# Dylan-H-Wang/skin-sm3

Measured on AMD Instinct MI355X. Metric: SM3 pretrain images/sec (paired 224x224), higher is better.
Workload: dtype bf16

## Files before the change

include/sm3_hip.h:

```cpp
#ifndef SM3_HIP_H
#define SM3_HIP_H

#include <stdint.h>

#ifdef __cplusplus
extern "C" {
#endif

#define SM3_F32 0
#define SM3_BF16 1
#define SM3_F16 2

#define SM3_EINVAL (-1)
#define SM3_EALIGN (-2)
#define SM3_EDTYPE (-3)

#define SM3_MAX_TAPS 9

int sm3_abi_version(void);

typedef struct sm3_conv_desc {
    int32_t dtype;
    int32_t N, Hi, Wi, Ci;
    int32_t Ho, Wo, Co;
// ... 68 lines not shown
                    float* save_invstd , void* stream);
int sm3_bn_eval_scale_shift(const float* gamma, const float* beta, const float* running_mean,
                            const float* running_var, float eps, int C, float* scale, float* shift,
                            void* stream);
int sm3_bn_act(int dtype, const void* x, const float* scale, const float* shift, const void* residual,
               int relu, int out_f32, void* y, uint8_t* relu_mask, int64_t rows, int C, int views, void* stream);
int sm3_bn_act_colsum_rows(int64_t rows, int C, int dtype);
int sm3_bn_act_colsum(int dtype, const void* x, const float* scale, const float* shift, const void* residual, int relu,
                      void* y, uint8_t* relu_mask, float* colsum_partials, int64_t rows, int C, int views, void* stream);
int sm3_subsample_colsum_rows(int64_t rows, int C, int dtype);
int sm3_subsample_colsum(int dtype, const void* x, void* y, float* colsum_partials, int N, int H, int W, int C, int stride,
                         int views, void* stream);
int sm3_bn_add_bn_act(int dtype, const void* x, const float* scale, const float* shift, const void* x2,
                      const float* scale2, const float* shift2, int relu, void* y, uint8_t* relu_mask,
                      int64_t rows, int C, int views, void* stream);
int sm3_bn_bwd_partial_rows(int64_t rows, int C);
int sm3_bn_bwd_reduce(int dtype, const void* dy, const void* y, const uint8_t* relu_mask, const void* x,
                      const float* mean, const float* invstd, void* dz, int64_t rows, int C,
                      float* partials , int views, void* stream);
int sm3_bn_bwd_apply(int dtype, const void* dz, const void* x, const float* mean, const float* invstd,
                     const float* gamma, const double* global_sums, double count,
                     const double* local_sums, float* dgamma, float* dbeta, void* dx, int64_t rows,
                     int C, int views, void* stream);

typedef struct sm3_bn_apply_side {
    const void* x;
    const float* mean;
    const float* invstd;
    const float* gamma;
    const double* global_sums;
    const double* local_sums;
    float* dgamma;
    float* dbeta;
    void* dx;
} sm3_bn_apply_side;
int sm3_bn_bwd_apply2(int dtype, const void* dz, double count, const sm3_bn_apply_side* a,
                      const sm3_bn_apply_side* b, int64_t rows, int C, int views, void* stream);

int sm3_linbn_moments(const float* slabs, int nslabs, int64_t n, float* out, const float* colsum_partials, int colsum_rows,
                      double* s_out, int p, int views, void* stream);
int sm3_linbn_fwd_stats(int dtype, const float* G, const void* w_dgrad, const void* w_fwd, const double* s, float* Tm,
                        double* sums_ws, int C, int p, int views, void* stream);
int sm3_linbn_stats(int dtype, const float* P, const void* w_fwd, const float* mean, const float* invstd, const float* gamma,
                    const double* reduce_ws, int groups, double* lsums, float* dgamma, float* dbeta, double count,
                    float* coef, int C, int p, int views, void* stream);
int sm3_linbn_coef(const double* global_sums, double count, const float* gamma, const float* mean, const float* invstd,
// ... 232 lines not shown
```

skin-sm3_amd/csrc/bn.hip:

```cpp
#include "common.h"
#include <cstdlib>

namespace {

struct RowWalk {
    int tbx, tby;
    int gx, gy;
};
static RowWalk make_walk(int64_t rows, int cvecs, int max_gy, int views = 1) {
    RowWalk w;
    if (cvecs >= 256) {
        w.tbx = 256;
    } else {
        w.tbx = cvecs;
    }
    w.tby = 256 / w.tbx;
    if (w.tby < 1) w.tby = 1;
    w.gx = (cvecs + w.tbx - 1) / w.tbx;
    int64_t gy = (rows + (int64_t)w.tby * 8 - 1) / ((int64_t)w.tby * 8);
    static const int grid_cap = getenv("SM3_BN_GRID_CAP") ? atoi(getenv("SM3_BN_GRID_CAP")) : 768;
    const int64_t cap = grid_cap / (w.gx * views) > 0 ? grid_cap / (w.gx * views) : 1;
    if (gy > cap) gy = cap;
    if (gy > max_gy) gy = max_gy;
    if (gy < 1) gy = 1;
// ... 40 lines not shown
    double a = (a0 + a1) + (a2 + a3);
    a += __shfl_xor(a, 1, 64);
    a += __shfl_xor(a, 2, 64);
    return a;
}

__global__ void bn_stats_reduce_b(const double* __restrict__ ws, int G, int C, double* __restrict__ sums) {
    ws += (long)blockIdx.z * G * 2 * C;
    sums += (long)blockIdx.z * 2 * C;
    const int t = blockIdx.x * blockDim.x + threadIdx.x, q = t & 3;
    const int col = t >> 2;
    const double a = quad_sum_groups(ws, 2L * C, col < 2 * C ? col : 0, G, q);
    if (col < 2 * C && q == 0) sums[col] = a;
}

struct BnFinalizeArgs {
    double count;
    int C;
    const float *gamma, *beta;
    float eps, momentum;
    float *running_mean, *running_var;
    float *scale, *shift, *save_mean, *save_invstd;
};
__device__ __forceinline__ void bn_finalize_channel(const double* __restrict__ sums, int groups, int views, int c, int lane16,
                                                    const BnFinalizeArgs& a) {
    const int C = a.C;
    const int q = lane16 & 3, stat = (lane16 >> 2) & 1, vl = (lane16 >> 3) & 1;
    const int cc = c < C ? c : 0;
    float rm = 0.f, rv = 0.f;
    const bool owner = (c < C) && (lane16 == 0);
    if (owner) {
        rm = a.running_mean ? a.running_mean[c] : 0.f;
        rv = a.running_var ? a.running_var[c] : 0.f;
    }
    for (int v0 = 0; v0 < views; v0 += 2) {
        const int v = v0 + vl;
        const bool vok = v < views;
        const double* sv = sums + (long)(vok ? v : v0) * groups * 2 * C;
        const double mine = quad_sum_groups(sv, 2L * C, (long)stat * C + cc, groups, q);
        const double s2_same_view = __shfl_down(mine, 4, 64);
        const double s1_v1 = __shfl_down(mine, 8, 64);
        const double s2_v1 = __shfl_down(mine, 12, 64);
        if (!owner) continue;
        for (int k = 0; k < 2 && v0 + k < views; ++k) {
            const double s1 = k ? s1_v1 : mine, s2 = k ? s2_v1 : s2_same_view;
            const int vv = v0 + k;
            const double mean = s1 / a.count;
            double var = s2 / a.count - mean * mean;
            if (var < 0) var = 0;
            const double invstd = 1.0 / sqrt(var + (double)a.eps);
            const float g = a.gamma ? a.gamma[c] : 1.f, b = a.beta ? a.beta[c] : 0.f;
            a.scale[(long)vv * C + c] = (float)(g * invstd);
            a.shift[(long)vv * C + c] = (float)((double)b - mean * (double)g * invstd);
            if (a.save_mean) a.save_mean[(long)vv * C + c] = (float)mean;
            if (a.save_invstd) a.save_invstd[(long)vv * C + c] = (float)invstd;
            rm = (1.f - a.momentum) * rm + a.momentum * (float)mean;
            const double unbiased = var * (a.count / fmax(a.count - 1.0, 1.0));
            rv = (1.f - a.momentum) * rv + a.momentum * (float)unbiased;
        }
    }
    if (owner) {
        if (a.running_mean) a.running_mean[c] = rm;
        if (a.running_var) a.running_var[c] = rv;
    }
}

__global__ void bn_finalize_kernel(const double* __restrict__ sums, int groups, int views, int64_t* nbt, BnFinalizeArgs a) {
    const int t = blockIdx.x * blockDim.x + threadIdx.x;
    if (t == 0 && nbt) nbt[0] += views;
    bn_finalize_channel(sums, groups, views, t >> 4, t & 15, a);
}

__global__ void bn_eval_kernel(const float* gamma, const float* beta, const float* rm, const float* rv, float eps,
                               int C, float* scale, float* shift) {
    const int c = blockIdx.x * blockDim.x + threadIdx.x;
    if (c >= C) return;
    const float invstd = 1.f / sqrtf(rv[c] + eps);
    const float g = gamma ? gamma[c] : 1.f, b = beta ? beta[c] : 0.f;
    scale[c] = g * invstd;
    shift[c] = b - rm[c] * g * invstd;
}
// ... 427 lines not shown
        for (int e = 0; e < E; ++e) o[e] = k0a[e] * (g[e] - k1a[e]) - (xv[e] - mua[e]) * qa[e];
        stg16<NT>(dxa + r * C + (int64_t)cv * E, pack16<T>(o));
        unpack16<T>(xbu, xv);
#pragma unroll
        for (int e = 0; e < E; ++e) o[e] = k0b[e] * (g[e] - k1b[e]) - (xv[e] - mub[e]) * qb[e];
        stg16<NT>(dxb + r * C + (int64_t)cv * E, pack16<T>(o));
    };
    int64_t r = (int64_t)blockIdx.y * tby + ty;
    for (; r + (U - 1) * rstep < rows; r += U * rstep) {
        uint4 gu[U], xau[U], xbu[U];
#pragma unroll
        for (int u = 0; u < U; ++u) {
            const int64_t off = (r + u * rstep) * C + (int64_t)cv * E;
            gu[u] = ldg16<NT>(dz + off);
            xau[u] = ldg16<NT>(xa + off);
            xbu[u] = ldg16<NT>(xb + off);
        }
#pragma unroll
        for (int u = 0; u < U; ++u) finish(r + u * rstep, gu[u], xau[u], xbu[u]);
    }
    for (; r < rows; r += rstep) {
        const int64_t off = r * C + (int64_t)cv * E;
        finish(r, ldg16<false>(dz + off), ldg16<false>(xa + off), ldg16<false>(xb + off));
    }
}

static int env_int(const char* name, int dflt) {
    const char* v = getenv(name);
    return v && *v ? atoi(v) : dflt;
}
static int bn_unroll(int kind) {
    static const int u[3] = {env_int("SM3_BN_UNROLL_ACT", env_int("SM3_BN_UNROLL", 4)),
                             env_int("SM3_BN_UNROLL_RED", env_int("SM3_BN_UNROLL", 4)),
                             env_int("SM3_BN_UNROLL_APP", env_int("SM3_BN_UNROLL", 8))};
    return u[kind];
}
static bool bn_nt() {
    static const bool nt = env_int("SM3_BN_NT", 1) != 0;
    return nt;
}
#define SM3_BN_DISPATCH(KIND, CALL)                 \
    do {                                            \
        const int u_ = bn_unroll(KIND);             \
        if (bn_nt()) {                              \
            if (u_ >= 8) { CALL(8, true); }         \
            else if (u_ >= 4) { CALL(4, true); }    \
// ... 209 lines not shown
    for (const sm3_bn_apply_side* s : {a, b})
        if (!s->x || !s->mean || !s->invstd || !s->global_sums || !s->dx) return SM3_EINVAL;
    if (!SM3_DTYPE_OK(dtype)) return SM3_EDTYPE;
    const int E = dtype == SM3_F32 ? 4 : 8;
    if (C % E) return SM3_EALIGN;
    const RowWalk w = make_walk(rows, C / E, 8192, views);
    dim3 grid(w.gx, w.gy, views), block(256);
    hipStream_t st = (hipStream_t)stream;
    const BnApplySide sa = {a->x, a->mean, a->invstd, a->gamma, a->global_sums, a->local_sums, a->dgamma, a->dbeta, a->dx};
    const BnApplySide sb = {b->x, b->mean, b->invstd, b->gamma, b->global_sums, b->local_sums, b->dgamma, b->dbeta, b->dx};
#define SM3_APP2_T(T, U, NT)                                                                                   \
    hipLaunchKernelGGL((bn_bwd_apply2_kernel<T, (U > 4 ? 4 : U), NT>), grid, block, 0, st, (const T*)dz, sa, sb,  \
                       1.0 / count, rows, C, w.tbx, w.tby)
#define SM3_APP2(U, NT)                                        \
    if (dtype == SM3_F32) { SM3_APP2_T(float, U, NT); }        \
    else if (dtype == SM3_BF16) { SM3_APP2_T(bf16_t, U, NT); } \
    else { SM3_APP2_T(f16_t, U, NT); }
    SM3_BN_DISPATCH(2, SM3_APP2);
#undef SM3_APP2
#undef SM3_APP2_T
    SM3_CHECK_LAUNCH();
    return 0;
}
```

skin-sm3_amd/sm3hip/_lib.py:

```python
import ctypes as C
import os

_HERE = os.path.dirname(os.path.abspath(__file__))
LIB_PATH = os.environ.get("SM3_LIBRARY") or os.path.join(_HERE, "libsm3hip.so")

SM3_F32, SM3_BF16, SM3_F16 = 0, 1, 2
MAX_TAPS = 9


class ConvDesc(C.Structure):
    _fields_ = [
        ("dtype", C.c_int32),
        ("N", C.c_int32), ("Hi", C.c_int32), ("Wi", C.c_int32), ("Ci", C.c_int32),
        ("Ho", C.c_int32), ("Wo", C.c_int32), ("Co", C.c_int32),
        ("sy", C.c_int32), ("sx", C.c_int32),
        ("ntaps", C.c_int32),
        ("dy", C.c_int32 * MAX_TAPS), ("dx", C.c_int32 * MAX_TAPS), ("wtap", C.c_int32 * MAX_TAPS),
        ("w_row_stride", C.c_int32),
        ("Hout", C.c_int32), ("Wout", C.c_int32),
        ("osy", C.c_int32), ("osx", C.c_int32), ("ooy", C.c_int32), ("oox", C.c_int32),
    ]


class BnBwdFuse(C.Structure):
# ... 52 lines not shown
    "sm3_linbn_stats": [_I, _P, _P, _P, _P, _P, _P, _I, _P, _P, _P, _D, _P, _I, _I, _I, _P],
    "sm3_linbn_coef": [_P, _D, _P, _P, _P, _P, _I, _I, _P],
    "sm3_linbn_banks": [_I, _P, _P, _P, _P, _P, _I, _I, _I, _P],
    "sm3_linbn_post": [_I, _P, _P, _P, _P, _P, _P, _P, _P, _P, _I, _I, _I, _P],
    "sm3_linbn_banks_post": [_I, _P, _P, _P, _P, _P, _P, _P, _P, _P, _P, _I, _I, _I, _P],
    "sm3_conv_bn_act_eval": [_DESC, _P, _P, _P, _P, _P, _I, _P, _P],
    "sm3_conv_bn_eval": [_DESC, _P, _P, _P, _P, _P, _P, _F, _P, _I, _P, _P],
    "sm3_conv_wgrad": [_DESC, _P, _P, _P, _P],
    "sm3_conv_wgrad_det": [_DESC, _P, _P, _P, _P, _I, _P],
    "sm3_slab_reduce": [_P, _I, _L, _P, _I, _P],
    "sm3_bn_stats_reduce": [_P, _I, _I, _P, _P, _I, _P],
    "sm3_bn_reduce_groups": [_I],
    "sm3_bn_finalize": [_P, _I, _I, _D, _I, _P, _P, _F, _F, _P, _P, _P, _P, _P, _P, _P, _P],
    "sm3_bn_eval_scale_shift": [_P, _P, _P, _P, _F, _I, _P, _P, _P],
    "sm3_bn_act": [_I, _P, _P, _P, _P, _I, _I, _P, _P, _L, _I, _I, _P],
    "sm3_bn_add_bn_act": [_I, _P, _P, _P, _P, _P, _P, _I, _P, _P, _L, _I, _I, _P],
    "sm3_bn_bwd_apply2": [_I, _P, _D, _P, _P, _L, _I, _I, _P],
    "sm3_bn_relu_maxpool_fwd": [_I, _P, _P, _P, _P, _P, _I, _I, _I, _I, _I, _P],
    "sm3_maxpool_bn_bwd_partial_rows": [_I, _I, _I, _I],
    "sm3_maxpool_bn_bwd": [_I, _P, _P, _P, _P, _P, _P, _P, _P, _P, _I, _I, _I, _I, _I, _P],
    "sm3_bn_bwd_partial_rows": [_L, _I],
    "sm3_bn_bwd_reduce": [_I, _P, _P, _P, _P, _P, _P, _P, _L, _I, _P, _I, _P],
    "sm3_bn_bwd_apply": [_I, _P, _P, _P, _P, _P, _P, _D, _P, _P, _P, _P, _L, _I, _I, _P],
    "sm3_stem_partial_rows": [_I, _I, _I],
    "sm3_stem_weight_prep": [_I, _P, _P, _P],
    "sm3_stem_weight_prep_if": [_I, _P, _P, _P, _P],
    "sm3_stem_conv_fwd": [_I, _P, _P, _P, _P, _I, _I, _I, _P],
    "sm3_stem_wgrad_bn": [_I, _P, _P, _P, _P, _P, _P, _P, _D, _P, _P, _P, _P, _P, _I, _I, _I, _I, _P],
    "sm3_stem_image_cols": [_I],
    "sm3_stem_image_prep": [_I, _P, _P, _P, _I, _I, _I, _I, _P],
    "sm3_stem_conv_fwd16": [_I, _P, _P, _P, _P, _I, _I, _I, _P],
    "sm3_stem_wgrad_bn16": [_I, _P, _P, _P, _P, _P, _P, _P, _D, _P, _P, _P, _P, _P, _I, _I, _I, _I, _P],
    "sm3_stem_dgrad_bn": [_I, _P, _P, _P, _P, _P, _P, _D, _P, _P, _I, _I, _I, _I, _P],
    "sm3_maxpool3x3s2_fwd": [_I, _P, _P, _P, _I, _I, _I, _I, _P],
    "sm3_maxpool3x3s2_bwd": [_I, _P, _P, _P, _I, _I, _I, _I, _P],
    "sm3_weight_prep_batch": [_I, _P, _I, _P],
    "sm3_weight_prep_batch_if": [_I, _P, _I, _P, _P],
    "sm3_weights_changed": [_P, _L, _P, _P, _P],
    "sm3_avgpool_fwd": [_I, _P, _P, _P, _I, _I, _I, _P],
    "sm3_avgpool_bwd": [_I, _P, _P, _I, _I, _I, _P],
    "sm3_weight_prep": [_I, _P, _I, _I, _I, _P, _I, _P, _P],
    "sm3_cast_from_f32": [_I, _P, _P, _L, _P],
    "sm3_cast_to_f32": [_I, _P, _P, _L, _P],
    "sm3_ntxent_logits": [_P, _I, _I, _F, _P, _P, _P, _P],
    "sm3_ntxent_logits_bwd": [_I, _P, _P, _P, _I, _I, _F, _P, _P],
    "sm3_ce_label0": [_P, _I, _I, _F, _P, _P, _P, _P],
# ... 106 lines not shown
```

skin-sm3_amd/sm3hip/engine.py:

```python
import os
from collections import OrderedDict
from contextlib import contextmanager

import torch

from . import ops
from ._lib import SM3_BF16, SM3_F16
from .plan import (TWO_PASS, BlockRec, EncoderCtx, ParamStore, ProjectorPlan, Rec, block_form, enc_mod_out_dim, enc_plan,
                   stage_of)
from .plan import EncoderPlan

BN_EPS = 1e-5
BN_MOMENTUM = 0.1


_LANE_POOL = {}


def lane_stream_pool(device, n):
    idx = device.index if device.index is not None else torch.cuda.current_device()
    pool = _LANE_POOL.setdefault(idx, [])
    if len(pool) >= n:
        return pool[:n]
    if os.environ.get("SM3_STREAM_CALIBRATE", "1") == "0" or not hasattr(torch.cuda, "_sleep"):
# ... 74 lines not shown
        self._lane = "main"
        self._V = 1
        self._data_only = False
        self._no_stat_update = False
        self.weights_dirty = True
        self._wprep_cache, self._wprep_key, self._hash_tracks_banks = {}, None, False
        self._lane_prep = {}
        self._lin_descs = {}
        self.last_feats = None
        self._faith_saved_bytes = {}
        self.pair_views = os.environ.get("SM3_PAIR_VIEWS", "1") != "0"
        self.two_streams = True
        self._streams, self._streams_dev = None, None
        self.linbn = self.dtype in (SM3_BF16, SM3_F16) and os.environ.get("SM3_LINBN", "1") != "0"
        self.linbn_fwd = os.environ.get("SM3_LINBN_FWD", "1") != "0"
        self.linbn_ds = os.environ.get("SM3_LINBN_DS", "1") != "0"
        self.linbn_join = os.environ.get("SM3_LINBN_JOIN", "1") != "0"
        self.linbn_merge = os.environ.get("SM3_LINBN_MERGE", "1") != "0"
        self.lane_cross = os.environ.get("SM3_LANE_CROSS", "1") != "0"
        if self.cross is not None and self.cross[0] is self.cross[1]:
            self.lane_cross = False
        self.det_wgrad = os.environ.get("SM3_WGRAD_DET", "1") != "0"
        self.stem16 = self.dtype in (SM3_BF16, SM3_F16) and os.environ.get("SM3_STEM16", "1") != "0"

    def _all_conv_units(self):
        seen = set()
        plans = [p for pair in self.branches.values() for p in pair if p is not None]
        plans += list(self.cross or ())
        if self.meta is not None:
            plans.append(self.meta)
        for plan in plans:
            for cu in plan.conv_units():
                if id(cu) not in seen:
                    seen.add(id(cu))
                    yield cu

    def prepare(self, device):
        if self.store is None or self.store.flat_p.device != device:
            self.store = ParamStore(self.module, device)
            self._allocated = False
        else:
            self.store.rebind_if_needed()
        if not self._allocated:
            for cu in self._all_conv_units():
                cu.alloc(self.dtype, device)
            self._allocated = True
# ... 130 lines not shown
            rm, rv = self.buffers[bu.name + ".running_mean"], self.buffers[bu.name + ".running_var"]
            nbt = self.buffers[bu.name + ".num_batches_tracked"]
        ops.bn_finalize(sums, count, bu.C, gamma, beta, BN_EPS, BN_MOMENTUM, rm, rv, nbt, scale, shift, mean, invstd,
                        groups=groups, views=V)

    @contextmanager
    def _views(self, V):
        self._V = V
        try:
            yield
        finally:
            self._V = 1

    @contextmanager
    def _params_backward(self, params):
        prev = self._data_only
        self._data_only = prev or not params
        try:
            yield
        finally:
            self._data_only = prev

    def conv_bn(self, cu, bu, x, N, H, W, relu, residual=None, train=True, save=False, out_f32=False, y_out=None,
                apply=True, scale_shift=None, res_affine=None, pending=None, colsum=None):
        dev = x.t.device if isinstance(x, ops.StemImage) else x.device
        direct = cu.stem
        if direct:
            d = None
            Ho, Wo = (H - 1) // 2 + 1, (W - 1) // 2 + 1
        else:
            d = cu.fwd_desc(self.dtype, N, H, W)
            Ho, Wo = d.Ho, d.Wo
        rows = N * Ho * Wo
        C = cu.Co
        V = self._V if train else 1
        rows_v = rows // V
        xo = torch.empty(rows, C, dtype=self.tdt, device=dev)
        scale, shift = scale_shift if scale_shift is not None else (self._work("scale", 2 * 2048),
                                                                    self._work("shift", 2 * 2048))
        mean = invstd = None

        def convolve(partials):
            if direct:
                (ops.stem_conv_fwd16 if isinstance(x, ops.StemImage) else ops.stem_conv_fwd)(self.dtype, x, cu.w_fwd, xo, partials)
            elif cu.groups > 1:
                ops.gconv_fwd(self.dtype, x, cu.w_fwd, xo, partials, N, H, W, C, cu.groups, cu.stride)
            else:
                ops.conv_gemm(d, x, cu.w_fwd, xo, None, partials)
        if train:
            prow = ops.stem_partial_rows(N, H, W) if direct else ops.conv_partial_rows(d)
            if V > 1 and ((rows_v % 128 and not direct) or prow % V):
                raise ValueError("two views in one batch need a multiple of 128 rows per view")
            partials = self._work("partials", prow * 2 * C)
            convolve(partials)
            count, groups = rows_v, 1
            mean = torch.empty(V * C, dtype=torch.float32, device=dev)
            invstd = torch.empty(V * C, dtype=torch.float32, device=dev)
            deferred = False
            if self.stat_sync is not None:
                count = rows_v * self.world_size
                n = V * 2 * C
                if pending is not None and not apply:
                    pair = self._work("sums_pair", 2 * 2 * 2 * 2048, torch.float64)
                    sums = pair[:n]
                    ops.bn_stats_reduce(partials, prow // V, C, sums, views=V)
                    deferred = True
                elif pending:
                    pair = self._work("sums_pair", 2 * 2 * 2 * 2048, torch.float64)
                    n0 = pending[0][0]
                    sums = pair[n0:n0 + n]
                    ops.bn_stats_reduce(partials, prow // V, C, sums, views=V)
                    self.stat_sync(pair[: n0 + n])
                    for _, fin in pending:
                        fin()
                    del pending[:]
                else:
                    sums = self._work("sums", 2 * 2 * 2048, torch.float64)
# ... 23 lines not shown
        mask = None
        if not apply:
            y_out = None
        else:
            if y_out is None:
                y_out = torch.empty(rows, C, dtype=torch.float32 if out_f32 else self.tdt, device=dev)
            if save and relu:
                mask = torch.empty(rows * C // (16 // ops._sz(self.dtype)), dtype=torch.uint8, device=dev)
            cs = None
            if res_affine is not None:
                ops.bn_add_bn_act(self.dtype, xo, scale, shift, residual, res_affine[0], res_affine[1], relu, y_out,
                                  rows_v, C, mask=mask, views=V)
            else:
                if colsum is not None and save and train and not out_f32:
                    cs = colsum
                ops.bn_act(self.dtype, xo, scale, shift, residual, relu, y_out, rows_v, C, out_f32=out_f32, mask=mask,
                           views=V, colsum=cs)
        r = None
        if save:
            r = Rec(cu, bu, N, H, W, Ho, Wo, x_in=x, xo=xo, mean=mean, invstd=invstd, y=y_out, relu=relu, mask=mask, V=V,
                    frozen_stats=not train, colsum=cs if apply else None)
        return (y_out if apply else xo), Ho, Wo, r

    def _phase1(self, r, dy, fused_rows):
        if fused_rows is not None:
            return fused_rows, self._ws[(self._lane, "fz_partials")]
        C, V = r.cu.Co, r.V
        rows = r.N * r.Ho * r.Wo // V
        prow = ops.bn_bwd_partial_rows(rows, C)
        bpart = self._work("partials", V * prow * 2 * C)
        ops.bn_bwd_reduce(self.dtype, dy, None, r.xo, r.mean, r.invstd, dy if r.relu else None, rows, C, bpart,
                          mask=r.mask if r.relu else None, views=V)
        return prow, bpart

    def bn_backward(self, r, dy, keep_dz, fused_rows=None):
        C = r.cu.Co
        V = r.V
        rows = r.xo.shape[0] // V
        prow, bpart = self._phase1(r, dy, fused_rows)
        lsums, gsums, count = self._bn_backward_sums(r, bpart, prow)
        dxo = torch.empty_like(r.xo) if keep_dz else dy
        dgamma, dbeta = self._bn_affine(r.bu, grad=True)
        ops.bn_bwd_apply(self.dtype, dy, r.xo, r.mean, r.invstd, self._bn_affine(r.bu)[0], gsums, count, lsums, dgamma, dbeta,
                         dxo, rows, C, views=V)
        return dxo, dy

    def _bn_backward_sums(self, r, bpart, prow):
        C, V = r.cu.Co, r.V
        rows = r.xo.shape[0] // V
        lsums = self._work("lsums", 2 * 2 * 2048, torch.float64)
        ops.bn_stats_reduce(bpart, prow, C, lsums, views=V)
        gsums, count = lsums, rows
        if r.frozen_stats:
            gsums = self._work("zsums", 2 * 2 * 2048, torch.float64)
            gsums.zero_()
        elif self.stat_sync is not None:
            gsums = self._work("gsums", 2 * 2 * 2048, torch.float64)
            gsums[: V * 2 * C].copy_(lsums[: V * 2 * C])
            self.stat_sync(gsums[: V * 2 * C])
            count = rows * self.world_size
        return lsums, gsums, count
# ... 500 lines not shown
            dd = cd.compact_dgrad_desc(self.dtype, rd.N, rd.Ho, rd.Wo)
            if cd.stride == 2:
                dsp = torch.empty(rd.N * rd.Ho * rd.Wo, Cin, dtype=self.tdt, device=dcur.device)
                ops.conv_gemm_seg(dd, dcur, dxd["wa"], dxd["x1"], dxd["hn"], dxd["const"], dsp, None, views=rd.V,
                                  w_view_stride=Cin * Cd, w1_view_stride=Cin * Cin)
                return self.conv_backward(r1, dx1, addend=dsp, fuse=prev, addend_sparse=(rd.Ho, rd.Wo))
            din, _ = self.conv_backward(r1, dx1)
            ops.conv_gemm_seg(dd, dcur, dxd["wa"], dxd["x1"], dxd["hn"], dxd["const"], din, din, views=rd.V,
                              w_view_stride=Cin * Cd, w1_view_stride=Cin * Cin)
            return din, None
        if br.form.sparse_join and prev is not None:
            self._wgrad(cd, rd, dxd)
            hs, ws = rd.Ho, rd.Wo
            dd = cd.compact_dgrad_desc(self.dtype, rd.N, hs, ws)
            dsp = torch.empty(rd.N * hs * ws, cd.Ci, dtype=self.tdt, device=dxd.device)
            ops.conv_gemm(dd, dxd, cd.w_dgrad, dsp, None, None)
            return self.conv_backward(r1, dx1, addend=dsp, fuse=prev, addend_sparse=(hs, ws))
        din, _ = self.conv_backward(r1, dx1)
        self.conv_backward(rd, dxd, into=din)
        return din, None

    def projector_forward(self, plan, x_t, M, train, z_out, save=None):
        saving = save is not None
        h, _, _, r0 = self.conv_bn(plan.l0, plan.b1, x_t, M, 1, 1, True, None, train, saving)
        h, _, _, r3 = self.conv_bn(plan.l3, plan.b4, h, M, 1, 1, True, None, train, saving)
        r6 = self.conv_bn(plan.l6, plan.b7, h, M, 1, 1, False, None, train, saving, out_f32=True, y_out=z_out)[3]
        if saving:
            save.append((r0, r3, r6))

    def projector_backward(self, recs, dz, addend=None, into=None):
        r0, r3, r6 = recs
        dx, _ = self.bn_backward(r6, dz, keep_dz=False)
        d, fr = self.conv_backward(r6, dx, fuse=r3)
        dx, _ = self.bn_backward(r3, d, keep_dz=False, fused_rows=fr)
        d, fr = self.conv_backward(r3, dx, fuse=r0)
        dx, _ = self.bn_backward(r0, d, keep_dz=False, fused_rows=fr)
        if into is not None:
            return self.conv_backward(r0, dx, into=into)[0]
        return self.conv_backward(r0, dx, addend=addend)[0]

    @staticmethod
    def cross_pairs(style):
        return {0: [(0, 0), (1, 1)], 1: [(0, 1), (1, 0)], 2: [(0, 0), (0, 1), (1, 0), (1, 1)]}[style]

    def forward(self, views, style=0, train=True, want_grad=True, metadata=None):
        first = next(iter(views.values()))[0]
        dev = first.device
        self.prepare(dev)
        self.refresh_weights(defer_lanes=self._lane_streams(dev) is not None and self.lane_cross)
        B = first.shape[0]
        saved = {"B": B, "style": style} if want_grad else None
        sv = (lambda: []) if want_grad else (lambda: None)
        zs, feats = OrderedDict(), {}
        streams = self._lane_streams(dev)
        lane_cross = self._cross_in_lanes(streams)
        pairs = self.cross_pairs(style) if self.cross is not None else []
        zc = [self._share(torch.empty(2 * B, self.module.proj_dim, dtype=torch.float32, device=dev), streams) for _ in pairs] \
            if lane_cross else []
        cross_recs = {}
# ... 178 lines not shown
```

skin-sm3_amd/sm3hip/ops.py:

```python
import ctypes as C

import torch

from . import _lib
from ._lib import ConvDesc, SM3_BF16, SM3_F16, SM3_F32, check

TORCH_DTYPE = {SM3_F32: torch.float32, SM3_BF16: torch.bfloat16, SM3_F16: torch.float16}
K_CHUNK = {SM3_F32: 32, SM3_BF16: 64, SM3_F16: 64}


_PROFILER = None


def set_profiler(p):
    global _PROFILER
    _PROFILER = p


class _prof:
    __slots__ = ("tag", "flops", "nbytes", "start")

    def __init__(self, tag, flops=0.0, nbytes=0.0):
        self.tag, self.flops, self.nbytes, self.start = tag, flops, nbytes, None

# ... 975 lines not shown
        check(_lib.load().sm3_bn_bwd_reduce(dtype, _ptr(dy), _ptr(y), _ptr(mask), _ptr(x), _ptr(mean), _ptr(invstd),
                                            _ptr(dz), rows, Cn, _ptr(partials), views, _stream()), "sm3_bn_bwd_reduce")


def bn_bwd_apply(dtype, dz, x, mean, invstd, gamma, gsums, count, lsums, dgamma, dbeta, dx, rows, Cn, views=1):
    tdt = TORCH_DTYPE[dtype]
    for t, n in ((dz, "dz"), (x, "x"), (dx, "dx")):
        _chk(t, tdt, n)
        if t.numel() != views * rows * Cn:
            raise ValueError(f"bn_bwd_apply: {n} size mismatch")
    _chk(gsums, torch.float64); _chk(lsums, torch.float64)
    _chk(dgamma, torch.float32); _chk(dbeta, torch.float32); _chk(gamma, torch.float32)
    if gsums.numel() < views * 2 * Cn or (lsums is not None and lsums.numel() < views * 2 * Cn):
        raise ValueError("bn_bwd_apply: sums too small")
    tag = "bn_bwd_apply"
    if _PROFILER is not None and getattr(_PROFILER, "detail", False):
        tag += f"|rows{views * rows}_C{Cn}"
    with _prof(tag, 0.0, _sz(dtype) * views * rows * Cn * 3):
        check(_lib.load().sm3_bn_bwd_apply(dtype, _ptr(dz), _ptr(x), _ptr(mean), _ptr(invstd), _ptr(gamma),
                                           _ptr(gsums), float(count), _ptr(lsums), _ptr(dgamma), _ptr(dbeta), _ptr(dx),
                                           rows, Cn, views, _stream()), "sm3_bn_bwd_apply")


STEM_KDIRECT = 176


def stem_partial_rows(N, H, W):
    return _lib.load().sm3_stem_partial_rows(N, H, W)


def stem_weight_prep(dtype, w_master, w_stem, only_if=None):
    _chk(w_master, torch.float32, "w_master"); _chk(w_stem, TORCH_DTYPE[dtype], "w_stem"); _chk(only_if, torch.int32, "only_if")
    if w_master.numel() != 64 * 147 or w_stem.numel() != 64 * STEM_KDIRECT:
        raise ValueError("stem_weight_prep: size mismatch")
    check(_lib.load().sm3_stem_weight_prep_if(dtype, _ptr(w_master), _ptr(w_stem), _ptr(only_if), _stream()),
          "sm3_stem_weight_prep_if")


def stem_conv_fwd(dtype, x_nchw, w_stem, y, partials=None):
    _chk(x_nchw, torch.float32, "x"); _chk(w_stem, TORCH_DTYPE[dtype], "w_stem"); _chk(y, TORCH_DTYPE[dtype], "y")
    _chk(partials, torch.float32, "partials")
    N, Cc, H, W = x_nchw.shape
    Ho, Wo = (H - 1) // 2 + 1, (W - 1) // 2 + 1
    if Cc != 3 or w_stem.numel() != 64 * STEM_KDIRECT or y.numel() != N * Ho * Wo * 64:
        raise ValueError("stem_conv_fwd: size mismatch")
    if partials is not None and partials.numel() < stem_partial_rows(N, H, W) * 2 * 64:
# ... 865 lines not shown
```

Before: 4680.

## Fuse projector BatchNorm1d stats finalize and apply into single-kernel tails

Adds single-launch BatchNorm1d forward and backward tail kernels for the small-row projector layers. Each kernel reduces the GEMM-produced partial sums, finalizes the statistics and applies the normalization (or gradient) in one launch, replacing the multi-kernel reduce/finalize/apply chain. The backward path has a self-summing variant for when no fused partials exist. This cuts launch overhead and extra global round trips for small tensors, at the cost of a narrow grid (C/32 blocks) and redundant per-block partial summation. It also adds atomics on dgamma/dbeta.

```diff
diff --git a/include/sm3_hip.h b/include/sm3_hip.h
--- a/include/sm3_hip.h
+++ b/include/sm3_hip.h
@@ -114,6 +114,14 @@
                      const float* gamma, const double* global_sums, double count,
                      const double* local_sums, float* dgamma, float* dbeta, void* dx, int64_t rows,
                      int C, int views, void* stream);
+
+int sm3_bn1d_fwd_tail(int dtype, const void* x, const float* partials, int partial_rows, int C, const float* gamma,
+                      const float* beta, float eps, float momentum, float* running_mean, float* running_var,
+                      int64_t* num_batches_tracked, float* save_mean, float* save_invstd, int relu, int out_f32, void* y,
+                      uint8_t* relu_mask, int64_t rows, void* stream);
+int sm3_bn1d_bwd_tail(int dtype, const void* dz, const void* x, const float* mean, const float* invstd, const float* gamma,
+                      const float* partials, int partial_rows, float* dgamma, float* dbeta, void* dx, int64_t rows, int C,
+                      void* stream);
 
 typedef struct sm3_bn_apply_side {
     const void* x;
diff --git a/skin-sm3_amd/csrc/bn.hip b/skin-sm3_amd/csrc/bn.hip
--- a/skin-sm3_amd/csrc/bn.hip
+++ b/skin-sm3_amd/csrc/bn.hip
@@ -86,6 +86,27 @@
     float *running_mean, *running_var;
     float *scale, *shift, *save_mean, *save_invstd;
 };
+struct BnViewStats {
+    float scale, shift, mean, invstd;
+};
+__device__ __forceinline__ BnViewStats bn_finalize_view(double s1, double s2, int c, const BnFinalizeArgs& a, float& rm,
+                                                        float& rv) {
+    const double mean = s1 / a.count;
+    double var = s2 / a.count - mean * mean;
+    if (var < 0) var = 0;
+    const double invstd = 1.0 / sqrt(var + (double)a.eps);
+    const float g = a.gamma ? a.gamma[c] : 1.f, b = a.beta ? a.beta[c] : 0.f;
+    BnViewStats o;
+    o.scale = (float)(g * invstd);
+    o.shift = (float)((double)b - mean * (double)g * invstd);
+    o.mean = (float)mean;
+    o.invstd = (float)invstd;
+    rm = (1.f - a.momentum) * rm + a.momentum * (float)mean;
+    const double unbiased = var * (a.count / fmax(a.count - 1.0, 1.0));
+    rv = (1.f - a.momentum) * rv + a.momentum * (float)unbiased;
+    return o;
+}
+
 __device__ __forceinline__ void bn_finalize_channel(const double* __restrict__ sums, int groups, int views, int c, int lane16,
                                                     const BnFinalizeArgs& a) {
     const int C = a.C;
@@ -109,18 +130,11 @@
         for (int k = 0; k < 2 && v0 + k < views; ++k) {
             const double s1 = k ? s1_v1 : mine, s2 = k ? s2_v1 : s2_same_view;
             const int vv = v0 + k;
-            const double mean = s1 / a.count;
-            double var = s2 / a.count - mean * mean;
-            if (var < 0) var = 0;
-            const double invstd = 1.0 / sqrt(var + (double)a.eps);
-            const float g = a.gamma ? a.gamma[c] : 1.f, b = a.beta ? a.beta[c] : 0.f;
-            a.scale[(long)vv * C + c] = (float)(g * invstd);
-            a.shift[(long)vv * C + c] = (float)((double)b - mean * (double)g * invstd);
-            if (a.save_mean) a.save_mean[(long)vv * C + c] = (float)mean;
-            if (a.save_invstd) a.save_invstd[(long)vv * C + c] = (float)invstd;
-            rm = (1.f - a.momentum) * rm + a.momentum * (float)mean;
-            const double unbiased = var * (a.count / fmax(a.count - 1.0, 1.0));
-            rv = (1.f - a.momentum) * rv + a.momentum * (float)unbiased;
+            const BnViewStats o = bn_finalize_view(s1, s2, c, a, rm, rv);
+            a.scale[(long)vv * C + c] = o.scale;
+            a.shift[(long)vv * C + c] = o.shift;
+            if (a.save_mean) a.save_mean[(long)vv * C + c] = o.mean;
+            if (a.save_invstd) a.save_invstd[(long)vv * C + c] = o.invstd;
         }
     }
     if (owner) {
@@ -594,6 +608,216 @@
     for (; r < rows; r += rstep) {
         const int64_t off = r * C + (int64_t)cv * E;
         finish(r, ldg16<false>(dz + off), ldg16<false>(xa + off), ldg16<false>(xb + off));
+    }
+}
+
+constexpr int kTailMaxPartialRows = 32;
+constexpr int kTailMaxSelfLanes = 512;
+
+template <typename P>
+__device__ __forceinline__ double tail_sum_rows(P p, int rows, long stride) {
+    double red[4];
+#pragma unroll
+    for (int ty = 0; ty < 4; ++ty) {
+        double a = 0.0, a1 = 0.0, a2 = 0.0, a3 = 0.0;
+        int r = ty;
+        for (; r + 12 < rows; r += 16) {
+            a += (double)p[(long)r * stride];
+            a1 += (double)p[(long)(r + 4) * stride];
+            a2 += (double)p[(long)(r + 8) * stride];
+            a3 += (double)p[(long)(r + 12) * stride];
+        }
+        for (; r < rows; r += 4) a += (double)p[(long)r * stride];
+        red[ty] = (a + a1) + (a2 + a3);
+    }
+    return (red[0] + red[1]) + (red[2] + red[3]);
+}
+
+template <typename T, bool OUT_F32>
+__global__ __launch_bounds__(256) void bn1d_fwd_tail_kernel(const T* __restrict__ x, const float* __restrict__ partials,
+                                                            int prow, int relu, void* __restrict__ y,
+                                                            uint8_t* __restrict__ mask, int rows, int C, int64_t* nbt,
+                                                            BnFinalizeArgs a) {
+    constexpr int E = ElemTraits<T>::kPer16B, VS = 4, CS = VS * E, RL = 256 / VS, U = 4;
+    __shared__ double ssum[2][CS];
+    __shared__ float ssc[CS], ssh[CS];
+    const int t = threadIdx.x, tx = t % VS, ty = t / VS;
+    const int c0 = blockIdx.x * CS, cv = blockIdx.x * VS + tx;
+    const bool active = cv * E < C;
+    uint4 xu[U];
+#pragma unroll
+    for (int u = 0; u < U; ++u) {
+        const int r = ty + u * RL;
+        xu[u] = (active && r < rows) ? ldg16<false>(x + (int64_t)r * C + (int64_t)cv * E) : make_uint4(0, 0, 0, 0);
+    }
+    if (t < 2 * CS) {
+        const int stat = t / CS, c = c0 + t % CS;
+        if (c < C) ssum[stat][t % CS] = tail_sum_rows(partials + (long)stat * C + c, prow, 2L * C);
+    }
+    if (blockIdx.x == 0 && t == 0 && nbt) nbt[0] += 1;
+    __syncthreads();
+    if (t < CS && c0 + t < C) {
+        const int c = c0 + t;
+        float rm = a.running_mean ? a.running_mean[c] : 0.f, rv = a.running_var ? a.running_var[c] : 0.f;
+        const BnViewStats o = bn_finalize_view(ssum[0][t], ssum[1][t], c, a, rm, rv);
+        ssc[t] = o.scale;
+        ssh[t] = o.shift;
+        if (a.save_mean) a.save_mean[c] = o.mean;
+        if (a.save_invstd) a.save_invstd[c] = o.invstd;
+        if (a.running_mean) a.running_mean[c] = rm;
+        if (a.running_var) a.running_var[c] = rv;
+    }
+    __syncthreads();
+    if (!active) return;
+    float sc[E], sh[E];
+#pragma unroll
+    for (int e = 0; e < E; ++e) {
+        sc[e] = ssc[tx * E + e];
+        sh[e] = ssh[tx * E + e];
+    }
+    auto finish = [&](int r, const uint4& xv) {
+        const int64_t off = (int64_t)r * C + (int64_t)cv * E;
+        float v[E];
+        unpack16<T>(xv, v);
+#pragma unroll
+        for (int e = 0; e < E; ++e) v[e] = v[e] * sc[e] + sh[e];
+        if (relu) {
+            if (mask) {
+                constexpr float thr = OUT_F32 ? 0.f : ElemTraits<T>::kReluBit;
+                unsigned m = 0;
+#pragma unroll
+                for (int e = 0; e < E; ++e) m |= (v[e] > thr ? 1u : 0u) << e;
+                mask[(int64_t)r * (C / E) + cv] = (uint8_t)m;
+            }
+#pragma unroll
+            for (int e = 0; e < E; ++e) v[e] = relu_f32(v[e]);
+        }
+        if constexpr (OUT_F32) {
+            float* yo = reinterpret_cast<float*>(y) + off;
+#pragma unroll
+            for (int e = 0; e < E; e += 4)
+                *reinterpret_cast<float4*>(yo + e) = make_float4(v[e], v[e + 1], v[e + 2], v[e + 3]);
+        } else {
+            stg16<false>(reinterpret_cast<T*>(y) + off, pack16<T>(v));
+        }
+    };
+#pragma unroll
+    for (int u = 0; u < U; ++u)
+        if (ty + u * RL < rows) finish(ty + u * RL, xu[u]);
+    for (int r = ty + U * RL; r < rows; r += RL) finish(r, ldg16<false>(x + (int64_t)r * C + (int64_t)cv * E));
+}
+
+template <typename T, int VS, bool SELF>
+__global__ __launch_bounds__(256) void bn1d_bwd_tail_kernel(const T* __restrict__ dz, const T* __restrict__ x,
+                                                            const float* __restrict__ mean,
+                                                            const float* __restrict__ invstd,
+                                                            const float* __restrict__ gamma,
+                                                            const float* __restrict__ partials, int prow,
+                                                            double inv_count, float* dgamma, float* dbeta, T* dx,
+                                                            int rows, int C, int tby, int gy) {
+    constexpr int E = ElemTraits<T>::kPer16B, CS = VS * E, RL = 256 / VS, U = 4;
+    static_assert(!SELF || VS == 1, "the self-summing form stages one vector per workgroup");
+    __shared__ double ssum[2][CS];
+    __shared__ float stage[SELF ? kTailMaxSelfLanes * 2 * E : 1];
+    __shared__ float sprow[SELF ? kTailMaxPartialRows * 2 * E : 1];
+    const int t = threadIdx.x, tx = t % VS, ty = t / VS;
+    const int c0 = blockIdx.x * CS, cv = blockIdx.x * VS + tx;
+    const bool active = cv * E < C;
+    float mu[E], is[E];
+#pragma unroll
+    for (int e = 0; e < E; ++e) {
+        mu[e] = active ? mean[cv * E + e] : 0.f;
+        is[e] = active ? invstd[cv * E + e] : 0.f;
+    }
+    uint4 gu[U], xu[U];
+    if constexpr (!SELF) {
+#pragma unroll
+        for (int u = 0; u < U; ++u) {
+            const int r = ty + u * RL;
+            const bool ok = active && r < rows;
+            const int64_t off = (int64_t)r * C + (int64_t)cv * E;
+            gu[u] = ok ? ldg16<false>(dz + off) : make_uint4(0, 0, 0, 0);
+            xu[u] = ok ? ldg16<false>(x + off) : make_uint4(0, 0, 0, 0);
+        }
+        if (t < 2 * CS) {
+            const int stat = t / CS, c = c0 + t % CS;
+            if (c < C) ssum[stat][t % CS] = tail_sum_rows(partials + (long)stat * C + c, prow, 2L * C);
+        }
+    } else {
+        const int rstep = gy * tby;
+        for (int p = t; p < rstep; p += 256) {
+            float s1[E], s2[E];
+#pragma unroll
+            for (int e = 0; e < E; ++e) s1[e] = s2[e] = 0.f;
+            for (int r = p; r < rows; r += rstep) {
+                const int64_t off = (int64_t)r * C + (int64_t)cv * E;
+                float g[E], xv[E];
+                unpack16<T>(ldg16<false>(dz + off), g);
+                unpack16<T>(ldg16<false>(x + off), xv);
+#pragma unroll
+                for (int e = 0; e < E; ++e) {
+                    s1[e] += g[e];
+                    s2[e] += g[e] * (xv[e] - mu[e]) * is[e];
+                }
+            }
+#pragma unroll
+            for (int e = 0; e < E; ++e) {
+                stage[p * 2 * E + e] = s1[e];
+                stage[p * 2 * E + E + e] = s2[e];
+            }
+        }
+        __syncthreads();
+        for (int i = t; i < gy * 2 * E; i += 256) {
+            const int by = i / (2 * E), j = i % (2 * E);
+            float acc = stage[(by * tby) * 2 * E + j];
+            for (int l = 1; l < tby; ++l) acc += stage[(by * tby + l) * 2 * E + j];
+            sprow[i] = acc;
+        }
+        __syncthreads();
+        if (t < 2 * E) ssum[t / E][t % E] = tail_sum_rows(sprow + t, gy, 2L * E);
+    }
+    __syncthreads();
+    if (!active) return;
+    float k0[E], k1[E], q[E];
+#pragma unroll
+    for (int e = 0; e < E; ++e) {
+        const float g = gamma ? gamma[cv * E + e] : 1.f;
+        k0[e] = g * is[e];
+        k1[e] = (float)(ssum[0][tx * E + e] * inv_count);
+        q[e] = k0[e] * is[e] * (float)(ssum[1][tx * E + e] * inv_count);
+    }
+    if (ty == 0) {
+        float db[E], dg[E];
+#pragma unroll
+        for (int e = 0; e < E; ++e) {
+            db[e] = dg[e] = 0.f;
+            db[e] += (float)ssum[0][tx * E + e];
+            dg[e] += (float)ssum[1][tx * E + e];
+        }
+#pragma unroll
+        for (int e = 0; e < E; ++e) {
+            if (dbeta) atomicAdd(&dbeta[cv * E + e], db[e]);
+            if (dgamma) atomicAdd(&dgamma[cv * E + e], dg[e]);
+        }
+    }
+    auto finish = [&](int r, const uint4& gv, const uint4& xv_) {
+        float g[E], xv[E];
+        unpack16<T>(gv, g);
+        unpack16<T>(xv_, xv);
+#pragma unroll
+        for (int e = 0; e < E; ++e) g[e] = k0[e] * (g[e] - k1[e]) - (xv[e] - mu[e]) * q[e];
+        stg16<false>(dx + (int64_t)r * C + (int64_t)cv * E, pack16<T>(g));
+    };
+    int r = ty;
+    if constexpr (!SELF) {
+#pragma unroll
+        for (int u = 0; u < U; ++u)
+            if (ty + u * RL < rows) finish(ty + u * RL, gu[u], xu[u]);
+        r = ty + U * RL;
+    }
+    for (; r < rows; r += RL) {
+        const int64_t off = (int64_t)r * C + (int64_t)cv * E;
+        finish(r, ldg16<false>(dz + off), ldg16<false>(x + off));
     }
 }
 
@@ -849,3 +1073,61 @@
     SM3_CHECK_LAUNCH();
     return 0;
 }
+
+static bool bn1d_rows_ok(int64_t rows) { return rows >= 128 && rows % 128 == 0 && rows <= 128 * kTailMaxPartialRows; }
+
+extern "C" int sm3_bn1d_fwd_tail(int dtype, const void* x, const float* partials, int partial_rows, int C,
+                                 const float* gamma, const float* beta, float eps, float momentum, float* running_mean,
+                                 float* running_var, int64_t* num_batches_tracked, float* save_mean, float* save_invstd,
+                                 int relu, int out_f32, void* y, uint8_t* relu_mask, int64_t rows, void* stream) {
+    if (!x || !partials || !y || C <= 0 || !bn1d_rows_ok(rows)) return SM3_EINVAL;
+    if (partial_rows < 1 || partial_rows > kTailMaxPartialRows || (relu_mask && !relu)) return SM3_EINVAL;
+    if (dtype != SM3_BF16 && dtype != SM3_F16) return SM3_EDTYPE;
+    if (C % 8) return SM3_EALIGN;
+    const BnFinalizeArgs a{(double)rows, C, gamma, beta, eps, momentum, running_mean, running_var, nullptr, nullptr, save_mean,
+                           save_invstd};
+    dim3 grid((C + 31) / 32), block(256);
+    hipStream_t st = (hipStream_t)stream;
+#define SM3_TAIL_F(T, F32)                                                                                              \
+    hipLaunchKernelGGL((bn1d_fwd_tail_kernel<T, F32>), grid, block, 0, st, (const T*)x, partials, partial_rows, relu, y,   \
+                       relu_mask, (int)rows, C, num_batches_tracked, a)
+    if (dtype == SM3_BF16) {
+        if (out_f32) SM3_TAIL_F(bf16_t, true); else SM3_TAIL_F(bf16_t, false);
+    } else {
+        if (out_f32) SM3_TAIL_F(f16_t, true); else SM3_TAIL_F(f16_t, false);
+    }
+#undef SM3_TAIL_F
+    SM3_CHECK_LAUNCH();
+    return 0;
+}
+
+extern "C" int sm3_bn1d_bwd_tail(int dtype, const void* dz, const void* x, const float* mean, const float* invstd,
+                                 const float* gamma, const float* partials, int partial_rows, float* dgamma, float* dbeta,
+                                 void* dx, int64_t rows, int C, void* stream) {
+    if (!dz || !x || !mean || !invstd || !dx || C <= 0 || !bn1d_rows_ok(rows)) return SM3_EINVAL;
+    if (partials && (partial_rows < 1 || partial_rows > kTailMaxPartialRows)) return SM3_EINVAL;
+    if (dtype != SM3_BF16 && dtype != SM3_F16) return SM3_EDTYPE;
+    if (C % 8) return SM3_EALIGN;
+    hipStream_t st = (hipStream_t)stream;
+    const double inv_count = 1.0 / (double)rows;
+    if (partials) {
+        dim3 grid((C + 31) / 32), block(256);
+#define SM3_TAIL_B(T)                                                                                                     \
+    hipLaunchKernelGGL((bn1d_bwd_tail_kernel<T, 4, false>), grid, block, 0, st, (const T*)dz, (const T*)x, mean, invstd,     \
+                       gamma, partials, partial_rows, inv_count, dgamma, dbeta, (T*)dx, (int)rows, C, 0, 0)
+        if (dtype == SM3_BF16) SM3_TAIL_B(bf16_t); else SM3_TAIL_B(f16_t);
+#undef SM3_TAIL_B
+    } else {
+        const RowWalk w = make_walk(rows, C / 8, 1 << 30);
+        const int gy = bwd_gy(rows);
+        if (gy > kTailMaxPartialRows || gy * w.tby > kTailMaxSelfLanes) return SM3_EINVAL;
+        dim3 grid(C / 8), block(256);
+#define SM3_TAIL_S(T)                                                                                                     \
+    hipLaunchKernelGGL((bn1d_bwd_tail_kernel<T, 1, true>), grid, block, 0, st, (const T*)dz, (const T*)x, mean, invstd,      \
+                       gamma, (const float*)nullptr, 0, inv_count, dgamma, dbeta, (T*)dx, (int)rows, C, w.tby, gy)
+        if (dtype == SM3_BF16) SM3_TAIL_S(bf16_t); else SM3_TAIL_S(f16_t);
+#undef SM3_TAIL_S
+    }
+    SM3_CHECK_LAUNCH();
+    return 0;
+}
diff --git a/skin-sm3_amd/sm3hip/_lib.py b/skin-sm3_amd/sm3hip/_lib.py
--- a/skin-sm3_amd/sm3hip/_lib.py
+++ b/skin-sm3_amd/sm3hip/_lib.py
@@ -98,6 +98,8 @@
     "sm3_bn_bwd_partial_rows": [_L, _I],
     "sm3_bn_bwd_reduce": [_I, _P, _P, _P, _P, _P, _P, _P, _L, _I, _P, _I, _P],
     "sm3_bn_bwd_apply": [_I, _P, _P, _P, _P, _P, _P, _D, _P, _P, _P, _P, _L, _I, _I, _P],
+    "sm3_bn1d_fwd_tail": [_I, _P, _P, _I, _I, _P, _P, _F, _F, _P, _P, _P, _P, _P, _I, _I, _P, _P, _L, _P],
+    "sm3_bn1d_bwd_tail": [_I, _P, _P, _P, _P, _P, _P, _I, _P, _P, _P, _L, _I, _P],
     "sm3_stem_partial_rows": [_I, _I, _I],
     "sm3_stem_weight_prep": [_I, _P, _P, _P],
     "sm3_stem_weight_prep_if": [_I, _P, _P, _P, _P],
diff --git a/skin-sm3_amd/sm3hip/engine.py b/skin-sm3_amd/sm3hip/engine.py
--- a/skin-sm3_amd/sm3hip/engine.py
+++ b/skin-sm3_amd/sm3hip/engine.py
@@ -120,6 +120,7 @@
             self.lane_cross = False
         self.det_wgrad = os.environ.get("SM3_WGRAD_DET", "1") != "0"
         self.stem16 = self.dtype in (SM3_BF16, SM3_F16) and os.environ.get("SM3_STEM16", "1") != "0"
+        self.proj_fused = self.dtype in (SM3_BF16, SM3_F16) and os.environ.get("SM3_PROJ_FUSED", "1") != "0"
 
     def _all_conv_units(self):
         seen = set()
@@ -296,7 +297,7 @@
             self._data_only = prev
 
     def conv_bn(self, cu, bu, x, N, H, W, relu, residual=None, train=True, save=False, out_f32=False, y_out=None,
-                apply=True, scale_shift=None, res_affine=None, pending=None, colsum=None):
+                apply=True, scale_shift=None, res_affine=None, pending=None, colsum=None, tail1d=False):
         dev = x.t.device if isinstance(x, ops.StemImage) else x.device
         direct = cu.stem
         if direct:
@@ -327,6 +328,9 @@
                 raise ValueError("two views in one batch need a multiple of 128 rows per view")
             partials = self._work("partials", prow * 2 * C)
             convolve(partials)
+            if tail1d and self._tail1d_ok(rows, C) and V == 1 and apply and residual is None and res_affine is None \
+                    and scale_shift is None and colsum is None and not direct and cu.groups == 1:
+                return self._bn1d_tail(cu, bu, x, xo, partials, prow, N, H, W, Ho, Wo, relu, save, out_f32, y_out)
             count, groups = rows_v, 1
             mean = torch.empty(V * C, dtype=torch.float32, device=dev)
             invstd = torch.empty(V * C, dtype=torch.float32, device=dev)
@@ -396,6 +400,27 @@
                     frozen_stats=not train, colsum=cs if apply else None)
         return (y_out if apply else xo), Ho, Wo, r
 
+    def _tail1d_ok(self, rows, C, self_sums=False):
+        return self.proj_fused and self.stat_sync is None and ops.bn1d_tail_ok(rows, C, self_sums)
+
+    def _bn1d_tail(self, cu, bu, x, xo, partials, prow, N, H, W, Ho, Wo, relu, save, out_f32, y_out):
+        rows, C, dev = xo.shape[0], cu.Co, xo.device
+        gamma, beta = self._bn_affine(bu)
+        rm = rv = nbt = None
+        if not self._no_stat_update:
+            rm, rv = self.buffers[bu.name + ".running_mean"], self.buffers[bu.name + ".running_var"]
+            nbt = self.buffers[bu.name + ".num_batches_tracked"]
+        mean = torch.empty(C, dtype=torch.float32, device=dev)
+        invstd = torch.empty(C, dtype=torch.float32, device=dev)
+        if y_out is None:
+            y_out = torch.empty(rows, C, dtype=torch.float32 if out_f32 else self.tdt, device=dev)
+        mask = torch.empty(rows * C // 8, dtype=torch.uint8, device=dev) if save and relu else None
+        ops.bn1d_fwd_tail(self.dtype, xo, partials, prow, C, gamma, beta, BN_EPS, BN_MOMENTUM, rm, rv, nbt, mean, invstd, relu,
+                          y_out, rows, out_f32=out_f32, mask=mask)
+        r = Rec(cu, bu, N, H, W, Ho, Wo, x_in=x, xo=xo, mean=mean, invstd=invstd, y=y_out, relu=relu, mask=mask, V=1,
+                frozen_stats=False, colsum=None) if save else None
+        return y_out, Ho, Wo, r
+
     def _phase1(self, r, dy, fused_rows):
         if fused_rows is not None:
             return fused_rows, self._ws[(self._lane, "fz_partials")]
@@ -407,10 +432,17 @@
                           mask=r.mask if r.relu else None, views=V)
         return prow, bpart
 
-    def bn_backward(self, r, dy, keep_dz, fused_rows=None):
+    def bn_backward(self, r, dy, keep_dz, fused_rows=None, tail1d=False):
         C = r.cu.Co
         V = r.V
         rows = r.xo.shape[0] // V
+        if tail1d and V == 1 and not r.frozen_stats and not keep_dz and (fused_rows is not None or not r.relu) \
+                and self._tail1d_ok(rows, C, self_sums=fused_rows is None):
+            part = self._ws[(self._lane, "fz_partials")] if fused_rows is not None else None
+            dgamma, dbeta = self._bn_affine(r.bu, grad=True)
+            ops.bn1d_bwd_tail(self.dtype, dy, r.xo, r.mean, r.invstd, self._bn_affine(r.bu)[0], part, fused_rows, dgamma, dbeta,
+                              dy, rows, C)
+            return dy, dy
         prow, bpart = self._phase1(r, dy, fused_rows)
         lsums, gsums, count = self._bn_backward_sums(r, bpart, prow)
         dxo = torch.empty_like(r.xo) if keep_dz else dy
@@ -957,19 +989,19 @@
 
     def projector_forward(self, plan, x_t, M, train, z_out, save=None):
         saving = save is not None
-        h, _, _, r0 = self.conv_bn(plan.l0, plan.b1, x_t, M, 1, 1, True, None, train, saving)
-        h, _, _, r3 = self.conv_bn(plan.l3, plan.b4, h, M, 1, 1, True, None, train, saving)
-        r6 = self.conv_bn(plan.l6, plan.b7, h, M, 1, 1, False, None, train, saving, out_f32=True, y_out=z_out)[3]
+        h, _, _, r0 = self.conv_bn(plan.l0, plan.b1, x_t, M, 1, 1, True, None, train, saving, tail1d=True)
+        h, _, _, r3 = self.conv_bn(plan.l3, plan.b4, h, M, 1, 1, True, None, train, saving, tail1d=True)
+        r6 = self.conv_bn(plan.l6, plan.b7, h, M, 1, 1, False, None, train, saving, out_f32=True, y_out=z_out, tail1d=True)[3]
         if saving:
             save.append((r0, r3, r6))
 
     def projector_backward(self, recs, dz, addend=None, into=None):
         r0, r3, r6 = recs
-        dx, _ = self.bn_backward(r6, dz, keep_dz=False)
+        dx, _ = self.bn_backward(r6, dz, keep_dz=False, tail1d=True)
         d, fr = self.conv_backward(r6, dx, fuse=r3)
-        dx, _ = self.bn_backward(r3, d, keep_dz=False, fused_rows=fr)
+        dx, _ = self.bn_backward(r3, d, keep_dz=False, fused_rows=fr, tail1d=True)
         d, fr = self.conv_backward(r3, dx, fuse=r0)
-        dx, _ = self.bn_backward(r0, d, keep_dz=False, fused_rows=fr)
+        dx, _ = self.bn_backward(r0, d, keep_dz=False, fused_rows=fr, tail1d=True)
         if into is not None:
             return self.conv_backward(r0, dx, into=into)[0]
         return self.conv_backward(r0, dx, addend=addend)[0]
diff --git a/skin-sm3_amd/sm3hip/ops.py b/skin-sm3_amd/sm3hip/ops.py
--- a/skin-sm3_amd/sm3hip/ops.py
+++ b/skin-sm3_amd/sm3hip/ops.py
@@ -1021,6 +1021,66 @@
                                            rows, Cn, views, _stream()), "sm3_bn_bwd_apply")
 
 
+BN1D_TAIL_MAX_ROWS = 4096
+
+
+def bn1d_tail_ok(rows, Cn, self_sums=False):
+    if rows < 128 or rows % 128 or rows > BN1D_TAIL_MAX_ROWS or Cn % 8:
+        return False
+    if self_sums:
+        gy = (rows + 63) // 64
+        return gy <= 32 and gy * max(1, 256 // min(Cn // 8, 256)) <= 512
+    return True
+
+
+def bn1d_fwd_tail(dtype, x, partials, prow, Cn, gamma, beta, eps, momentum, running_mean, running_var, nbt, save_mean,
+                  save_invstd, relu, y, rows, out_f32=False, mask=None):
+    tdt = TORCH_DTYPE[dtype]
+    _chk(x, tdt, "x"); _chk(y, torch.float32 if out_f32 else tdt, "y"); _chk(partials, torch.float32, "partials")
+    if x.numel() != rows * Cn or y.numel() != rows * Cn:
+        raise ValueError("bn1d_fwd_tail: size mismatch")
+    if partials.numel() < prow * 2 * Cn:
+        raise ValueError("bn1d_fwd_tail: partials too small")
+    for t, n in ((gamma, "gamma"), (beta, "beta"), (running_mean, "running_mean"), (running_var, "running_var"),
+                 (save_mean, "save_mean"), (save_invstd, "save_invstd")):
+        _chk(t, torch.float32, n)
+        if t is not None and t.numel() < Cn:
+            raise ValueError(f"bn1d_fwd_tail: {n} too small")
+    _chk(nbt, torch.int64, "num_batches_tracked"); _chk(mask, torch.uint8, "mask")
+    if mask is not None and (not relu or mask.numel() != rows * Cn // 8):
+        raise ValueError("bn1d_fwd_tail: mask needs relu and one byte per 8 elements")
+    tag = "bn1d_fwd_tail"
+    if _PROFILER is not None and getattr(_PROFILER, "detail", False):
+        tag += f"|rows{rows}_C{Cn}"
+    with _prof(tag, 0.0, (_sz(dtype) + (4 if out_f32 else _sz(dtype))) * rows * Cn):
+        check(_lib.load().sm3_bn1d_fwd_tail(dtype, _ptr(x), _ptr(partials), prow, Cn, _ptr(gamma), _ptr(beta), eps, momentum,
+                                            _ptr(running_mean), _ptr(running_var), _ptr(nbt), _ptr(save_mean),
+                                            _ptr(save_invstd), int(relu), int(out_f32), _ptr(y), _ptr(mask), rows, _stream()),
+              "sm3_bn1d_fwd_tail")
+
+
+def bn1d_bwd_tail(dtype, dz, x, mean, invstd, gamma, partials, prow, dgamma, dbeta, dx, rows, Cn):
+    tdt = TORCH_DTYPE[dtype]
+    for t, n in ((dz, "dz"), (x, "x"), (dx, "dx")):
+        _chk(t, tdt, n)
+        if t.numel() != rows * Cn:
+            raise ValueError(f"bn1d_bwd_tail: {n} size mismatch")
+    for t, n in ((mean, "mean"), (invstd, "invstd"), (gamma, "gamma"), (dgamma, "dgamma"), (dbeta, "dbeta")):
+        _chk(t, torch.float32, n)
+        if t is not None and t.numel() < Cn:
+            raise ValueError(f"bn1d_bwd_tail: {n} too small")
+    _chk(partials, torch.float32, "partials")
+    if partials is not None and partials.numel() < prow * 2 * Cn:
+        raise ValueError("bn1d_bwd_tail: partials too small")
+    tag = "bn1d_bwd_tail"
+    if _PROFILER is not None and getattr(_PROFILER, "detail", False):
+        tag += f"|rows{rows}_C{Cn}_self{int(partials is None)}"
+    with _prof(tag, 0.0, _sz(dtype) * rows * Cn * (3 if partials is not None else 5)):
+        check(_lib.load().sm3_bn1d_bwd_tail(dtype, _ptr(dz), _ptr(x), _ptr(mean), _ptr(invstd), _ptr(gamma), _ptr(partials),
+                                            prow if partials is not None else 0, _ptr(dgamma), _ptr(dbeta), _ptr(dx), rows,
+                                            Cn, _stream()), "sm3_bn1d_bwd_tail")
+
+
 STEM_KDIRECT = 176
 
 
```

New measurement: 4653. About the same (-0.6%).
